# buwantaiji/DominantSparseEigenAD

Hardware: AMD Instinct MI355X
Metric: DominantSparseSymeig fwd+bwd ms & HBM GB/s (TFIM, fp64) (higher is better)
Workload: dtype f64

## Files before the change

dominantsparseeigenad_amd/csrc/dsea_capi.hip:

```cpp
#include <hip/hip_runtime.h>
#include <stdint.h>
#include <stdlib.h>
#include <string.h>

#include <new>

#include "dsea_internal.h"

using namespace dsea;

namespace {
thread_local int g_last_hip = 0;

inline int64_t round_up(int64_t v, int64_t m) { return (v + m - 1) / m * m; }

struct WsLayout {
  size_t partials_off, aux_off, coef_off, scal_off, vec_off, total;
  int64_t npad;
};
WsLayout ws_layout(int64_t n, int kmax) {
  WsLayout L;
  const int kk = kmax < 1 ? 1 : kmax;
  L.npad = round_up(n < 1 ? 1 : n, 256);
  size_t off = 0;
// ... 316 lines not shown
  REQUIRE(rows >= 1 && ld >= 8 && tau >= 0.0, DSEA_ERR_ARG);
  REQUIRE(aligned16(shadow_bf16) && (ld % 8) == 0, DSEA_ERR_ALIGN);
  drop_shadow8(ws->w);
  ws->w.shadow = static_cast<uint16_t*>(shadow_bf16);
  ws->w.shadow_ld = ld;
  ws->w.shadow_rows = rows;
  ws->w.lp_tau = tau;
  return DSEA_OK;
}

int dsea_ws_set_shadow8(dsea_ws_t ws, void* shadow_e5m2, int64_t ld, int rows, double tau) {
  REQUIRE(ws, DSEA_ERR_ARG);
  if (!shadow_e5m2) {
    drop_shadow8(ws->w);
    return DSEA_OK;
  }
  REQUIRE(rows >= 1 && ld >= 16 && tau >= 0.0, DSEA_ERR_ARG);
  REQUIRE(aligned16(shadow_e5m2) && (ld % 16) == 0, DSEA_ERR_ALIGN);
  drop_shadow(ws->w);
  ws->w.shadow8 = static_cast<uint8_t*>(shadow_e5m2);
  ws->w.shadow8_ld = ld;
  ws->w.shadow8_rows = rows;
  ws->w.lp8_tau = tau;
  return DSEA_OK;
}

ShadowRow Workspace::shadow_row(int row, int64_t n_rows) const {
  if (shadow && shadow_rows > row && shadow_ld >= n_rows) return ShadowRow(shadow + (int64_t)row * shadow_ld);
  if (shadow8 && shadow8_rows > row && shadow8_ld >= n_rows)
    return ShadowRow(shadow8 + (int64_t)row * shadow8_ld, shadow8_scale(n_rows));
  return ShadowRow();
}

int dsea_lanczos_lp_stats(dsea_ws_t ws, int64_t* lp_steps, int64_t* fp64_steps, void* stream) {
  REQUIRE(ws && lp_steps && fp64_steps, DSEA_ERR_ARG);
  double h[2] = {0.0, 0.0};
  DSEA_TRY(read_to_host(h, ws->w.scal + 16, sizeof(h), static_cast<hipStream_t>(stream)));
  *lp_steps = (int64_t)h[0];
  *fp64_steps = (int64_t)h[1];
  return DSEA_OK;
}

int dsea_lanczos_reorth_stats(dsea_ws_t ws, int64_t* reorth_steps, double* anorm, void* stream) {
  REQUIRE(ws && reorth_steps, DSEA_ERR_ARG);
  double h[2] = {0.0, 0.0};
  DSEA_TRY(read_to_host(h, ws->w.scal + DSEA_SCAL_PRO + 2, sizeof(h), static_cast<hipStream_t>(stream)));
  if (anorm) *anorm = h[0];
  *reorth_steps = (int64_t)h[1];
  return DSEA_OK;
}

int dsea_ws_set_rows_per_lane(dsea_ws_t ws, int rpl) {
  REQUIRE(ws && (rpl == 0 || rpl == 2 || rpl == 4 || rpl == 8 || rpl == 16), DSEA_ERR_ARG);
  ws->w.rpl_override = rpl;
  return DSEA_OK;
}

int dsea_ws_set_persist(dsea_ws_t ws, int mode) {
  REQUIRE(ws, DSEA_ERR_ARG);
  if (mode == 200) {
    ws->w.persist_override = mode;
    return DSEA_OK;
  }
  const int geo = mode >= 100 ? mode - 100 : mode;
  REQUIRE(geo == -1 || geo == 0 || geo == 1 || geo == 2 || geo == 11 || geo == 12 || geo == 21 || geo == 22, DSEA_ERR_ARG);
  REQUIRE(mode < 100 || geo != -1, DSEA_ERR_ARG);
// ... 399 lines not shown
                     int64_t n, void* stream) {
  (void)ws;
  REQUIRE(r && nrm2 && q_out && n >= 1, DSEA_ERR_ARG);
  REQUIRE(aligned16(r) && aligned16(q_out), DSEA_ERR_ALIGN);
  launch_scale_store(r, nrm2, q_out, beta_out, n, static_cast<hipStream_t>(stream));
  return check_launch();
}

int dsea_lanczos_rdots(dsea_ws_t ws, const double* Q, int64_t ldq, int64_t n, int i, const double* u,
                       const double* alpha, const double* beta, double* r, double* c_out, void* stream) {
  REQUIRE(ws && Q && u && alpha && r && c_out && n >= 1 && i >= 1 && ldq >= n, DSEA_ERR_ARG);
  REQUIRE(i <= ws->w.kmax, DSEA_ERR_WORKSPACE);
  REQUIRE(aligned16(Q) && aligned16(u) && aligned16(r) && (ldq % 2 == 0), DSEA_ERR_ALIGN);
  TileGeom g = ws->w.geom(n);
  Profiler* prof = ws->w.prof;
  launch_rdots(g, Q, ldq, n, i, u, alpha, beta, r, ws->w.partials, c_out, static_cast<hipStream_t>(stream),
               prof ? prof->next(PROF_RDOTS) : nullptr, nullptr, 0, nullptr, true);
  return check_launch();
}

int dsea_lanczos_axpy_norm(dsea_ws_t ws, const double* Q, int64_t ldq, int64_t n, int i, const double* c,
                           double* r, double* nrm2_out, void* stream) {
  REQUIRE(ws && Q && c && r && nrm2_out && n >= 1 && i >= 1 && ldq >= n, DSEA_ERR_ARG);
  REQUIRE(aligned16(Q) && aligned16(r) && (ldq % 2 == 0), DSEA_ERR_ALIGN);
  hipStream_t st = static_cast<hipStream_t>(stream);
  Workspace& w = ws->w;
  if (w.shadow && w.shadow_rows >= i && w.shadow_ld >= n && !w.geom(n).split_w) {
    double* nP = w.aux + DSEA_MAX_WAVE_TILES;
    const int rps = lp_rows_per_step(n, false);
    int nn = launch_axpy_norm_lp(n, rps, Q, ldq, w.shadow, w.shadow_ld, i, c, w.lp_tau, r, nP, w.scal + 16, st);
    launch_finalize1(nP, nn, nrm2_out, st);
  } else if (w.shadow8 && w.shadow8_rows >= i && w.shadow8_ld >= n && lp8_applies(n, w.geom(n).split_w != 0)) {
    double* nP = w.aux + DSEA_MAX_WAVE_TILES;
    int nn = launch_axpy_norm_lp8(n, Q, ldq, w.shadow8, w.shadow8_ld, shadow8_scale(n), i, c, w.lp8_tau, r, nP, w.scal + 16, st);
    launch_finalize1(nP, nn, nrm2_out, st);
  } else {
    TileGeom g = w.geom(n);
    launch_axpy_norm(g, Q, ldq, n, i, c, r, w.partials, nrm2_out, st);
  }
  return check_launch();
}

int dsea_lanczos_partial_step(dsea_ws_t ws, const double* Q, int64_t ldq, int64_t n, int i, const double* u,
                              const double* alphas, const double* betas, double* r, double* nrm2_out, void* stream) {
  REQUIRE(ws && Q && u && alphas && betas && r && nrm2_out && n >= 1 && i >= 1 && ldq >= n, DSEA_ERR_ARG);
  REQUIRE(i <= ws->w.kmax, DSEA_ERR_WORKSPACE);
  REQUIRE(aligned16(Q) && aligned16(u) && aligned16(r) && (ldq % 2 == 0), DSEA_ERR_ALIGN);
  hipStream_t st = static_cast<hipStream_t>(stream);
  Workspace& w = ws->w;
  REQUIRE(w.n >= n, DSEA_ERR_WORKSPACE);
  const TileGeom g = w.geom(n);
  double* flag = w.scal + DSEA_SCAL_PRO;
  double* om = w.aux + 4 * DSEA_MAX_WAVE_TILES;
  if (i == 1) HIP_TRY(hipMemsetAsync(flag, 0, 4 * sizeof(double), st));
  launch_rdots(g, Q, ldq, n, i, u, alphas + (i - 1), i >= 2 ? betas + (i - 2) : nullptr, r, w.partials, nullptr, st, nullptr,
               nullptr, 0, nullptr, true, nullptr, w.zero, false);
  launch_pro_update(alphas, betas, w.partials + (int64_t)i * g.pstride, rdots_partial_count(g, i), w.coef + i, om,
                    DSEA_MAX_WAVE_TILES, flag, flag + 1, i, 64.0 * 2.220446049250313e-16, w.pro_delta, nullptr, st);
  launch_rdots(g, Q, ldq, n, i, r, w.zero, nullptr, w.vec[2], w.partials, w.coef, st, nullptr, nullptr, 0, nullptr, false,
               nullptr, flag, true);
  launch_axpy_norm(g, Q, ldq, n, i, w.coef, r, w.partials, nrm2_out, st, nullptr, nullptr, flag);
  return check_launch();
}

int dsea_lanczos_store(dsea_ws_t ws, const double* r, const double* nrm2, double* Q, int64_t ldq, int row,
                       double* beta_out, int64_t n, void* stream) {
  REQUIRE(ws && r && nrm2 && Q && n >= 1 && row >= 0 && ldq >= n, DSEA_ERR_ARG);
// ... 219 lines not shown

int dsea_lanczos_run(dsea_op_t op, dsea_ws_t ws, int k, const double* q0, double* Q, int64_t ldq,
                     double* alphas, double* betas, void* stream) {
  REQUIRE(op && ws && q0 && Q && alphas && betas && k >= 1, DSEA_ERR_ARG);
  const int64_t n = op->d.n;
  REQUIRE(ldq >= n && ws->w.n >= n, DSEA_ERR_ARG);
  REQUIRE(k <= ws->w.kmax || k == 1, DSEA_ERR_WORKSPACE);
  REQUIRE(aligned16(q0) && aligned16(Q) && (ldq % 2 == 0), DSEA_ERR_ALIGN);
  hipStream_t st = static_cast<hipStream_t>(stream);
  Workspace& w = ws->w;
  double* P = w.partials;
  double* u = w.vec[0];
  double* r = w.vec[1];
  double* nrm2 = w.scal + 0;
  TileGeom g = w.geom(n);

  Profiler* prof = w.prof;
  uint16_t* Qs = nullptr;
  int64_t lds = 0;
  if (!w.partial_reorth && w.shadow && w.shadow_rows >= k && w.shadow_ld >= n && (!w.geom(n).split_w || n >= 32768)) {
    Qs = w.shadow;
    lds = w.shadow_ld;
  }
  uint8_t* Qs8 = nullptr;
  if (!w.partial_reorth && w.shadow8 && w.shadow8_rows >= k && w.shadow8_ld >= n && lp8_applies(n, g.split_w != 0))
    Qs8 = w.shadow8;
  const int64_t ld8 = w.shadow8_ld;
  const double scale8 = shadow8_scale(n);
  const bool lp = Qs || Qs8;
  auto shadow_row = [&](int i) -> ShadowRow {
    if (Qs8) return ShadowRow(Qs8 + (int64_t)i * ld8, scale8);
    return ShadowRow(Qs ? Qs + (int64_t)i * lds : nullptr);
  };
  double* lp_count = w.scal + 16;
  double* brk = w.scal + DSEA_SCAL_BREAK;
  HIP_TRY(hipMemsetAsync(lp_count, 0, (DSEA_SCAL_BREAK + 2 - 16) * sizeof(double), st));
  HIP_TRY(hipMemsetAsync(w.scal + DSEA_SCAL_LZ_FAIL, 0, (DSEA_SCAL_PRO + 4 - DSEA_SCAL_LZ_FAIL) * sizeof(double), st));
  if (w.lz_persist != 0 && w.reorth_passes == 1 && !w.partial_reorth && (w.lz_persist == 1 || n <= 4096) && !prof && lanczos_persist_applicable(op->d, n, k) &&
      lanczos_persist_comm_bytes(n, k) <= w.partials_bytes()) {
    const int rc = persist_status(launch_lanczos_persist(op->d, k, q0, Q, ldq, alphas, betas, brk, w.scal + DSEA_SCAL_LZ_FAIL, P,
                                                         st, w.lose_peer));
    if (rc != PERSIST_SKIPPED) return rc == DSEA_OK ? check_launch() : rc;
  }
  if (w.lz_persist != 0 && w.lz_persist != 2 && (w.lz_persist == 1 || (n >= 49152 && k <= 400)) && w.reorth_passes == 1 &&
      !w.partial_reorth && !prof && lanczos_persist_mid_applicable(op->d, n, k) &&
      lanczos_persist_mid_comm_bytes(n, k) <= w.partials_bytes()) {
    const int rc = persist_status(launch_lanczos_persist_mid(op->d, k, q0, Q, ldq, Qs, lds, w.lp_tau, alphas, betas, brk,
                                                             w.scal + DSEA_SCAL_LZ_FAIL, lp_count, P, st, w.lose_peer));
    if (rc != PERSIST_SKIPPED) return rc == DSEA_OK ? check_launch() : rc;
  }
  const int rps = lp_rows_per_step(n, g.split_w != 0);
  const bool fused_tail = has_fused_tail(op->d);
  if (w.partial_reorth && !fused_tail) return DSEA_ERR_UNSUPPORTED;
  double* aP = w.aux;
  double* nP = w.aux + DSEA_MAX_WAVE_TILES;
  auto correct = [&](int i, double* fp64P, EventPair* ev, bool close) -> int {
    int nn = g.nw;
    if (Qs8)
      nn = launch_axpy_norm_lp8(n, Q, ldq, Qs8, ld8, scale8, i, w.coef, w.lp8_tau, r, nP, lp_count, st, ev, brk);
    else if (Qs)
      nn = launch_axpy_norm_lp(n, rps, Q, ldq, Qs, lds, i, w.coef, w.lp_tau, r, nP, lp_count, st, ev, brk);
    else
      launch_axpy_norm(g, Q, ldq, n, i, w.coef, r, fp64P, nullptr, st, ev, brk);
    if (close) launch_finalize_slot(lp ? nP : fp64P, nn, nrm2, brk, st);
    return nn;
  };
  auto second_pass = [&](int i, double* fp64P, bool close, int& nn) -> int {
    HIP_TRY(hipMemcpyAsync(w.vec[2], r, (size_t)n * sizeof(double), hipMemcpyDeviceToDevice, st));
    launch_rdots(g, Q, ldq, n, i, w.vec[2], w.zero, nullptr, r, P, w.coef, st, nullptr, nullptr, 0, nullptr, lp, brk);
    nn = correct(i, fp64P, nullptr, close);
    return DSEA_OK;
  };
  launch_dot(q0, q0, n, P, nrm2, st);
  launch_scale_store(q0, nrm2, Q, nullptr, n, st, shadow_row(0));
  if (fused_tail) {
    int na = launch_spmv(op->d, Q, u, nullptr, nullptr, aP, st, prof ? prof->next(PROF_SPMV) : nullptr);
    if (na < 0) return DSEA_ERR_UNSUPPORTED;
    double* pro_flag = w.scal + DSEA_SCAL_PRO;
    double* pro_om = w.aux + 4 * DSEA_MAX_WAVE_TILES;
    const double pro_eps1 = 64.0 * 2.220446049250313e-16;
    for (int i = 1; i < k; ++i) {
      const double* beta_prev = (i >= 2) ? betas + (i - 2) : nullptr;
      if (w.partial_reorth) {
        launch_rdots(g, Q, ldq, n, i, u, nullptr, beta_prev, r, P, nullptr, st, nullptr, aP, na, alphas + (i - 1),
                     true, brk, w.zero, false);
        launch_pro_update(alphas, betas, P + (int64_t)i * g.pstride, rdots_partial_count(g, i), w.coef + i, pro_om,
                          DSEA_MAX_WAVE_TILES, pro_flag, pro_flag + 1, i, pro_eps1, w.pro_delta, brk, st);
        launch_rdots(g, Q, ldq, n, i, r, w.zero, nullptr, w.vec[2], P, w.coef, st,
                     prof ? prof->next(PROF_RDOTS) : nullptr, nullptr, 0, nullptr, false, brk, pro_flag, true);
        launch_axpy_norm(g, Q, ldq, n, i, w.coef, r, nP, nullptr, st, prof ? prof->next(PROF_AXPY) : nullptr, brk, pro_flag);
        na = launch_tfim_fused(op->d, r, nP, g.nw, Q + (int64_t)i * ldq, u, betas + (i - 1), aP, st,
                               prof ? prof->next(PROF_SPMV) : nullptr, nullptr, brk, i);
        continue;
      }
      launch_rdots(g, Q, ldq, n, i, u, nullptr, beta_prev, r, P, w.coef, st,
                   prof ? prof->next(PROF_RDOTS) : nullptr, aP, na, alphas + (i - 1), lp, brk);
      int nn = correct(i, nP, prof ? prof->next(PROF_AXPY) : nullptr, false);
      if (w.reorth_passes == 2) DSEA_TRY(second_pass(i, nP, false, nn));
      na = launch_tfim_fused(op->d, r, nP, nn, Q + (int64_t)i * ldq, u, betas + (i - 1), aP, st,
                             prof ? prof->next(PROF_SPMV) : nullptr, shadow_row(i), brk, i);
    }
    launch_finalize_slot(aP, na, alphas + (k - 1), brk, st);
    return check_launch();
  }
  int nb = launch_spmv(op->d, Q, u, nullptr, nullptr, P, st, prof ? prof->next(PROF_SPMV) : nullptr);
  if (nb < 0) return DSEA_ERR_UNSUPPORTED;
  launch_finalize1(P, nb, alphas, st);
  for (int i = 1; i < k; ++i) {
    const double* beta_prev = (i >= 2) ? betas + (i - 2) : nullptr;
    launch_rdots(g, Q, ldq, n, i, u, alphas + (i - 1), beta_prev, r, P, w.coef, st,
                 prof ? prof->next(PROF_RDOTS) : nullptr, nullptr, 0, nullptr, lp, brk);
    int nn = correct(i, P, prof ? prof->next(PROF_AXPY) : nullptr, true);
    if (w.reorth_passes == 2) DSEA_TRY(second_pass(i, P, true, nn));
    double* qi = Q + (int64_t)i * ldq;
    launch_scale_store(r, nrm2, qi, betas + (i - 1), n, st, shadow_row(i), brk, i);
    nb = launch_spmv(op->d, qi, u, nullptr, brk, P, st, prof ? prof->next(PROF_SPMV) : nullptr);
    launch_finalize_slot(P, nb, alphas + i, brk, st);
  }
  return check_launch();
}

int dsea_lanczos_run_basisfree(dsea_op_t op, dsea_ws_t ws, int k, const double* q0, double* Qrot, int64_t ldq,
                               double* alphas, double* betas, const double* s, double* psi, void* stream) {
  REQUIRE(op && ws && q0 && Qrot && alphas && betas && k >= 1 && ((s == nullptr) == (psi == nullptr)), DSEA_ERR_ARG);
  const int64_t n = op->d.n;
  REQUIRE(ldq >= n && ws->w.n >= n, DSEA_ERR_ARG);
  REQUIRE(aligned16(q0) && aligned16(Qrot) && (!psi || aligned16(psi)) && (ldq % 2 == 0), DSEA_ERR_ALIGN);
  REQUIRE(has_fused_tail(op->d), DSEA_ERR_UNSUPPORTED);
  hipStream_t st = static_cast<hipStream_t>(stream);
  Workspace& w = ws->w;
  double* u = w.vec[0];
  double* r = w.vec[1];
  double* nrm2 = w.scal + 0;
  double* aP = w.aux;
  double* nP = w.aux + DSEA_MAX_WAVE_TILES;
  double* brk = w.scal + DSEA_SCAL_BREAK;
  HIP_TRY(hipMemsetAsync(brk, 0, 2 * sizeof(double), st));
  HIP_TRY(hipMemsetAsync(w.scal + DSEA_SCAL_LZ_FAIL, 0, sizeof(double), st));
  if (psi) HIP_TRY(hipMemsetAsync(psi, 0, (size_t)n * sizeof(double), st));
  auto slot = [&](int i) { return Qrot + (int64_t)(i % 3) * ldq; };
  launch_dot(q0, q0, n, w.partials, nrm2, st);
  launch_scale_store(q0, nrm2, slot(0), nullptr, n, st, nullptr);
  int na = launch_spmv(op->d, slot(0), u, nullptr, nullptr, aP, st);
  if (na < 0) return DSEA_ERR_UNSUPPORTED;
// ... 364 lines not shown
```

dominantsparseeigenad_amd/csrc/dsea_internal.h:

```cpp
#ifndef DSEA_INTERNAL_H
#define DSEA_INTERNAL_H

#include <hip/hip_ext.h>
#include <hip/hip_runtime.h>
#include <stdint.h>

#include <functional>
#include <type_traits>

#include "../../include/dsea.h"

#define DSEA_MAX_EW_BLOCKS 2048
#define DSEA_MAX_WAVE_TILES 8192
#define DSEA_TFIM_TILE_LOG2 11
#define DSEA_MAX_TFIM_BLOCKS 4096
#define DSEA_PERSIST_MAX_TILES 4096
#define DSEA_MAX_KRYLOV 8000
#define DSEA_PERSIST_CG_MAX_TILES 1024
#define DSEA_SCALARS 64
#define DSEA_SCAL_BREAK 20
#define DSEA_SCAL_PRO 40
#define DSEA_PRO_DELTA_DEFAULT 1e-10
#define DSEA_SCAL_LZ_FAIL 38

// ... 75 lines not shown
  const double* c;
};
struct LatticeDesc {
  int L, nb;
  const double* c;
  uint8_t a[DSEA_LATTICE_MAX_BONDS], b[DSEA_LATTICE_MAX_BONDS];
};
enum OpKind { OP_TFIM = 1, OP_CSR = 2, OP_STENCIL3 = 3, OP_SELL = 4, OP_DENSE = 5, OP_TRANSFER = 6, OP_SYMDENSE = 7, OP_CHAIN = 8,
              OP_LATTICE = 9 };
struct OpDesc {
  OpKind kind;
  int64_t n;
  int tune_tile_log2;
  int tune_csr_group;
  int tune_sell_unroll;
  TfimParams tfim;
  CsrParams csr;
  Stencil3Params st3;
  SellParams sell;
  DenseParams dense;
  TransferParams transfer;
  SymDenseParams symdense;
  ChainParams chain;
  LatticeDesc lattice;
};

struct ShadowRow {
  uint16_t* h;
  uint8_t* b;
  double S;
  ShadowRow(uint16_t* bf16 = nullptr) : h(bf16), b(nullptr), S(0.0) {}
  ShadowRow(uint8_t* e5m2, double scale) : h(nullptr), b(e5m2), S(scale) {}
};

struct TileGeom {
  int rpl;
  int nw;
  int64_t ntiles;
  int pstride;
  int split_w;
  int dots_w;
  int dots_nt;
};

template <int V>
using int_c = std::integral_constant<int, V>;
template <int V, int... Rest, class F>
inline void dispatch_int(int v, F&& f) {
  if constexpr (sizeof...(Rest) == 0) {
    f(int_c<V>{});
  } else {
    if (v == V) f(int_c<V>{});
    else dispatch_int<Rest...>(v, f);
  }
}
template <class F>
inline void dispatch_bool(bool b, F&& f) {
  if (b) f(std::true_type{});
  else f(std::false_type{});
}
template <class F>
inline void dispatch_rpl(int rpl, F&& f) { dispatch_int<2, 4, 8, 16>(rpl, f); }
template <class F>
inline void dispatch_split_w(int w, F&& f) { dispatch_int<4, 8, 16>(w, f); }

enum ProfKind { PROF_RDOTS = 0, PROF_AXPY = 1, PROF_SPMV = 2, PROF_KINDS = 3 };
// ... 19 lines not shown
  }
};

struct Workspace {
  int64_t n, npad;
  int kmax;
  int rpl_override;
  int split_override;
  int persist_override;
  int lz_persist;
  int arnoldi_optimistic;
  int last_cg_form;
  int lose_peer;
  int reorth_passes;
  int partial_reorth;
  double pro_delta;
  double* partials;
  double* aux;
  double* coef;
  double* coef2;
  double* zero;
  double* scal;
  double* vec[4];
  Profiler* prof;
  uint16_t* shadow;
  int64_t shadow_ld;
  int shadow_rows;
  double lp_tau;
  uint8_t* shadow8;
  int64_t shadow8_ld;
  int shadow8_rows;
  double lp8_tau;
  ShadowRow shadow_row(int row, int64_t n) const;
  int callable_na;
  int defer_norm;
  const double* pend_P;
  int pend_count;
  double* pend_out;
  TileGeom geom(int64_t n_rows) const;
  size_t partials_bytes() const { return (size_t)DSEA_MAX_WAVE_TILES * (size_t)((kmax < 1 ? 1 : kmax) + 1) * sizeof(double); }
  size_t aux_bytes() const { return (size_t)4 * DSEA_MAX_WAVE_TILES * sizeof(double); }
};

inline int ew_blocks(int64_t n) {
  int64_t nb = (n + 2047) / 2048;
  if (nb < 1) nb = 1;
  if (nb > DSEA_MAX_EW_BLOCKS) nb = DSEA_MAX_EW_BLOCKS;
  return (int)nb;
}
inline int tile_blocks(int64_t n) {
  const int64_t nt = (n + 511) / 512;
  return nt <= DSEA_PERSIST_MAX_TILES ? (int)(nt < 1 ? 1 : nt) : ew_blocks(n);
}

void launch_finalize1(const double* P, int count, double* out, hipStream_t st);
int launch_three_term(const double* u, const double* q1, const double* q2, const double* aP, int aCount,
                      double* a_store, const double* beta, double* r, double* P, double* psi, const double* s1,
                      int64_t n, double* brk, hipStream_t st);
void launch_finalize_slot(const double* P, int count, double* out, const double* skip, hipStream_t st);
void launch_rdots(const TileGeom& g, const double* Q, int64_t ldq, int64_t n, int i, const double* u,
                  const double* alpha, const double* beta, double* r, double* P, double* c_out,
                  hipStream_t st, EventPair* ev = nullptr, const double* aP = nullptr, int aCount = 0,
                  double* a_store = nullptr, bool want_rr = false, double* brk = nullptr,
                  const double* sel = nullptr, bool sel_exit = false, const double* uscale = nullptr);
inline bool rdots_uscale_ok(const TileGeom& g) { return g.split_w == 0; }
int launch_axpy_norm_lp(int64_t n, int rps, const double* Q, int64_t ldq, const uint16_t* Qs, int64_t lds, int i,
                        const double* c, double tau, double* r, double* P, double* lp_count, hipStream_t st,
                        EventPair* ev = nullptr, const double* brk = nullptr);
int launch_axpy_norm_lp8(int64_t n, const double* Q, int64_t ldq, const uint8_t* Qs8, int64_t ld8, double scale, int i,
                         const double* c, double tau, double* r, double* P, double* lp_count, hipStream_t st,
                         EventPair* ev = nullptr, const double* brk = nullptr);
inline double shadow8_scale(int64_t n) {
  int e = 0;
  while (e < 15 && ((int64_t)1 << (2 * e)) < n) ++e;
  return (double)((int64_t)1 << e);
}
int launch_tfim_fused(const OpDesc& op, const double* r, const double* nP, int nCount, double* q_out, double* y,
                      double* beta_store, double* P, hipStream_t st, EventPair* ev = nullptr,
                      ShadowRow qs_out = ShadowRow(), double* brk = nullptr, int step = 0);
int launch_cg_update_fused(double* x, double* r, const double* d, const double* Ad, const double* state,
                           int parity, const double* dP, int dCount, int64_t n, double* P, hipStream_t st);
void launch_cg_direction_fused(const double* r, double* d, double* state, int parity, const double* rP,
                               int rCount, double eps, int64_t n, hipStream_t st);
void launch_axpy_norm(const TileGeom& g, const double* Q, int64_t ldq, int64_t n, int i, const double* c,
                      double* r, double* P, double* nrm2_out, hipStream_t st, EventPair* ev = nullptr,
                      const double* brk = nullptr, const double* sel = nullptr);
void launch_ritz(const TileGeom& g, const double* Q, int64_t ldq, int64_t n, int k, const double* s,
                 double* out, hipStream_t st);
void launch_dot(const double* x, const double* y, int64_t n, double* P, double* out, hipStream_t st);
void launch_pro_update(const double* alphas, const double* betas, const double* rrP, int rrCount, double* rr_store,
                       double* om, int ld, double* flag, double* state, int i, double eps1, double delta,
                       const double* brk, hipStream_t st);
int rdots_partial_count(const TileGeom& g, int i);
void launch_probe(const double* x, double* y, int64_t n, double* P, int nP, hipStream_t st);
void launch_shift_dot(const double* x, double* y, const double* shift, const double* skip, int64_t n,
                      double* P, double* out, hipStream_t st);
int launch_shift_dot_partials(const double* x, double* y, const double* shift, const double* skip, int64_t n, double* P,
                              hipStream_t st);
void launch_axpy(double a_host, const double* a_dev, const double* x, double* y, int64_t n, hipStream_t st);
void launch_scale_store(const double* r, const double* nrm2, double* q, double* beta_out, int64_t n,
                        hipStream_t st, ShadowRow qs = ShadowRow(), double* brk = nullptr, int step = 0);
void launch_scale_store_fused(const double* r, const double* nP, int nCount, double* q, ShadowRow qs, double* beta_store,
                              int64_t n, hipStream_t st);
int launch_dot_partials(const double* x, const double* y, int64_t n, double* P, hipStream_t st);
// ... 150 lines not shown
```

dominantsparseeigenad_amd/csrc/dsea_lanczos_kernels.hip:

```cpp

#include <hip/hip_runtime.h>
#include <stdint.h>

#include "dsea_internal.h"
#include "dsea_device.h"

namespace dsea {

__global__ __launch_bounds__(256) void k_finalize1(const double* __restrict__ partials, int count,
                                                   double* __restrict__ out) {
  __shared__ double sm4[4];
  double acc = 0.0;
  for (int b = threadIdx.x; b < count; b += 256) acc += partials[b];
  double t = block_sum(acc, sm4);
  if (threadIdx.x == 0) out[0] = t;
}

void launch_finalize1(const double* P, int count, double* out, hipStream_t st) {
  hipLaunchKernelGGL(k_finalize1, dim3(1), dim3(256), 0, st, P, count, out);
}

__global__ __launch_bounds__(256) void k_finalize_pair(const double* __restrict__ PA, int na, double* __restrict__ outA,
                                                       const double* __restrict__ PB, int nb, double* __restrict__ outB,
                                                       const double* __restrict__ skipB) {
  __shared__ double sm4[4];
  const bool second = blockIdx.x == 1;
  if (second && skipB && skipB[0] != 0.0) return;
  const double* __restrict__ P = second ? PB : PA;
  const int count = second ? nb : na;
  double acc = 0.0;
  for (int b = threadIdx.x; b < count; b += 256) acc += P[b];
  double t = block_sum(acc, sm4);
  if (threadIdx.x == 0) (second ? outB : outA)[0] = t;
}

void launch_finalize_pair(const double* PA, int na, double* outA, const double* PB, int nb, double* outB,
                          const double* skipB, hipStream_t st) {
  hipLaunchKernelGGL(k_finalize_pair, dim3(2), dim3(256), 0, st, PA, na, outA, PB, nb, outB, skipB);
}

template <bool GATE>
__global__ __launch_bounds__(256) void k_finalize_multi(const double* __restrict__ P, int64_t pstride,
                                                        int nw, double* __restrict__ c,
                                                        const double* __restrict__ brk,
                                                        const double* __restrict__ gate) {
  __shared__ double sm4[4];
  const double gate0 = GATE ? gate[0] : 1.0;
  if (broken(brk)) return;
  if (GATE && gate0 == 0.0) return;
  const int j = blockIdx.x;
  const double* __restrict__ row = P + (int64_t)j * pstride;
  double a0 = 0.0, a1 = 0.0, a2 = 0.0, a3 = 0.0;
  int w = threadIdx.x;
  for (; w + 768 < nw; w += 1024) {
    a0 += row[w];
    a1 += row[w + 256];
    a2 += row[w + 512];
    a3 += row[w + 768];
  }
  for (; w < nw; w += 256) a0 += row[w];
  double t = block_sum((a0 + a1) + (a2 + a3), sm4);
  if (threadIdx.x == 0) c[j] = t;
}

template <int NP>
struct RdotsPre {
  double2 uu[NP], qa[NP], qb[NP];
};

template <int RPL, bool GUARD, bool PRE, bool USCALE = false>
__device__ __forceinline__ void rdots_tile(const double* __restrict__ Q, int64_t ldq, int i, int ii, int64_t n,
                                           int64_t base, int lane, const double* __restrict__ u,
                                           double a, double b, double* __restrict__ r,
                                           double* __restrict__ sP, bool accumulate, bool want_rr,
                                           const RdotsPre<RPL / 2>& pre, double usc = 1.0) {
  constexpr int NP = RPL / 2;
  double2 rv[NP];
  const double* __restrict__ q1 = Q + (int64_t)(i - 1) * ldq;
  const double* __restrict__ q2 = (i >= 2) ? Q + (int64_t)(i - 2) * ldq : nullptr;
#pragma unroll
  for (int t = 0; t < NP; ++t) {
    const int64_t row = base + t * 128 + lane * 2;
    double2 uu, qa, qb;
    if (PRE) {
      uu = pre.uu[t];
      qa = pre.qa[t];
      qb = pre.qb[t];
    } else {
      uu = ld2<GUARD>(u, row, n);
      qa = ld2<GUARD>(q1, row, n);
      qb = make_double2(0.0, 0.0);
      if (q2) qb = ld2<GUARD>(q2, row, n);
    }
    if (USCALE) {
      uu.x = uu.x / usc;
// ... 314 lines not shown
  part[wv][lane] = w;
  __syncthreads();
  if (wv == 0) {
    double2 tot = part[0][lane];
#pragma unroll
    for (int k2 = 1; k2 < W; ++k2) {
      tot.x += part[k2][lane].x;
      tot.y += part[k2][lane].y;
    }
    if (MODE == 0) {
      double2 rv = ld2<true>(r, row, n);
      rv.x -= tot.x;
      rv.y -= tot.y;
      st2<true>(r, row, n, rv);
      double acc = wave_sum(fma(rv.x, rv.x, rv.y * rv.y));
      if (lane == 0) P[tile] = acc;
    } else {
      st2<true>(r, row, n, tot);
    }
  }
}

static inline int rdots_waves_per_block(int i) { return (i + 1) <= 2048 ? 4 : ((i + 1) <= 4096 ? 2 : 1); }

int rdots_partial_count(const TileGeom& g, int i) {
  if (g.split_w) return (int)((g.ntiles + g.dots_nt - 1) / g.dots_nt);
  const int wpb = rdots_waves_per_block(i);
  return (g.nw + wpb - 1) / wpb;
}

void launch_rdots(const TileGeom& g, const double* Q, int64_t ldq, int64_t n, int i, const double* u,
                  const double* alpha, const double* beta, double* r, double* P, double* c_out,
                  hipStream_t st, EventPair* ev, const double* aP, int aCount, double* a_store, bool want_rr,
                  double* brk, const double* sel, bool sel_exit, const double* uscale) {
  const int wr = want_rr ? 1 : 0;
  const int count = rdots_partial_count(g, i);
  if (g.split_w) {
    const size_t lds = (size_t)(i + 1) * sizeof(double);
    auto go = [&](auto w, auto nt) {
      dispatch_bool(sel != nullptr, [&](auto s) {
        constexpr int W = decltype(w)::value;
        constexpr bool SEL = decltype(s)::value;
        klaunch(ev, k_rdots_split<W, decltype(nt)::value, SEL>, count, W * 64, lds, st, Q, ldq, i, n, u, alpha, beta, r,
                P, g.pstride, aP, aCount, a_store, wr, brk, sel, SEL && sel_exit ? 1 : 0);
      });
    };
    if (g.dots_nt == 2) go(int_c<16>{}, int_c<2>{});
    else dispatch_split_w(g.dots_w, [&](auto w) { go(w, int_c<1>{}); });
  } else {
    const int wpb = rdots_waves_per_block(i);
    const size_t lds = (size_t)wpb * (i + 1) * sizeof(double);
    dispatch_int<1, 2, 0>(sel ? 1 : (uscale ? 2 : 0), [&](auto variant) {
      dispatch_rpl(g.rpl, [&](auto rpl) {
        constexpr bool SEL = decltype(variant)::value == 1, USCALE = decltype(variant)::value == 2;
        klaunch(ev, k_rdots<decltype(rpl)::value, SEL, USCALE>, count, 64 * wpb, lds, st, Q, ldq, i, n, u, alpha, beta, r,
                P, g.pstride, g.nw, g.ntiles, aP, aCount, a_store, wr, brk, sel, !USCALE && sel_exit ? 1 : 0,
                USCALE ? uscale : nullptr);
      });
    });
  }
  if (c_out)
    dispatch_bool(sel_exit, [&](auto gate) {
      constexpr bool GATE = decltype(gate)::value;
      klaunch(nullptr, k_finalize_multi<GATE>, want_rr ? i + 1 : i, 256, 0, st, P, g.pstride, count, c_out, brk,
              GATE ? sel : nullptr);
    });
}

template <int MODE>
static void launch_axpy_family(const TileGeom& g, const double* Q, int64_t ldq, int64_t n, int i, const double* c,
                               double* r, double* P, hipStream_t st, EventPair* ev, const double* brk,
                               const double* sel) {
  auto go = [&](auto s) {
    constexpr bool SEL = decltype(s)::value;
    if (g.split_w)
      dispatch_split_w(g.split_w, [&](auto w) {
        constexpr int W = decltype(w)::value;
        klaunch(ev, k_axpy_norm_split<W, MODE, SEL>, (unsigned)g.ntiles, W * 64, 0, st, Q, ldq, i, n, c, r, P, brk, sel);
      });
    else
      dispatch_rpl(g.rpl, [&](auto rpl) {
        klaunch(ev, k_axpy_norm<decltype(rpl)::value, MODE, SEL>, (g.nw + 3) / 4, 256, 0, st, Q, ldq, i, n, c, r, P, g.nw,
                g.ntiles, brk, sel);
      });
  };
  if constexpr (MODE == 0) dispatch_bool(sel != nullptr, go);
  else go(std::false_type{});
}

void launch_axpy_norm(const TileGeom& g, const double* Q, int64_t ldq, int64_t n, int i, const double* c,
                      double* r, double* P, double* nrm2_out, hipStream_t st, EventPair* ev, const double* brk,
                      const double* sel) {
  launch_axpy_family<0>(g, Q, ldq, n, i, c, r, P, st, ev, brk, sel);
  if (nrm2_out) launch_finalize1(P, g.nw, nrm2_out, st);
}

void launch_ritz(const TileGeom& g, const double* Q, int64_t ldq, int64_t n, int k, const double* s,
                 double* out, hipStream_t st) {
// ... 195 lines not shown
      st2<true>(r, row + 2 * t, n, rv);
      acc = fma(rv.x, rv.x, acc);
      acc = fma(rv.y, rv.y, acc);
    }
    acc = wave_sum(acc);
    if (lane == 0) P[tile] = acc;
  }
}

int launch_axpy_norm_lp(int64_t n, int rps, const double* Q, int64_t ldq, const uint16_t* Qs, int64_t lds, int i,
                        const double* c, double tau, double* r, double* P, double* lp_count, hipStream_t st,
                        EventPair* ev, const double* brk) {
  if (rps == 0) {
    const int64_t nt = (n + 511) / 512;
    klaunch(ev, k_axpy_norm_lp_split<16>, (unsigned)nt, 1024, 0, st, Q, ldq, Qs, lds, i, n, c, tau * tau, r, P, lp_count, brk);
    return (int)nt;
  }
  const int64_t tile = 512 * (int64_t)rps;
  int64_t ntiles = (n + tile - 1) / tile;
  if (ntiles < 1) ntiles = 1;
  const int nw = (int)(ntiles < DSEA_MAX_WAVE_TILES ? ntiles : DSEA_MAX_WAVE_TILES);
  dispatch_int<1, 2>(rps, [&](auto rows) {
    klaunch(ev, k_axpy_norm_lp<decltype(rows)::value>, (nw + 3) / 4, 256, 0, st, Q, ldq, Qs, lds, i, n, c, tau * tau, r, P,
            nw, ntiles, lp_count, brk);
  });
  return nw;
}

typedef float dsea_v2f __attribute__((ext_vector_type(2)));
__device__ __forceinline__ void fma_e5m2x4(dsea_v2f& w01, dsea_v2f& w23, dsea_v2f ch, uint32_t x) {
  w01 = __builtin_elementwise_fma(ch, __builtin_amdgcn_cvt_pk_f32_bf8((int)x, false), w01);
  w23 = __builtin_elementwise_fma(ch, __builtin_amdgcn_cvt_pk_f32_bf8((int)x, true), w23);
}
template <int RPS, bool GUARD>
__device__ __forceinline__ double axpy_lp8_tile(const uint8_t* __restrict__ Qs8, int64_t ld8, int i, int64_t n, int64_t base,
                                                int lane, const double* __restrict__ c, double cs, double rnorm,
                                                double* __restrict__ r) {
  dsea_v2f w[RPS][8];
#pragma unroll
  for (int s = 0; s < RPS; ++s)
#pragma unroll
    for (int e = 0; e < 8; ++e) w[s][e] = (dsea_v2f)(0.0f);
#ifndef DSEA_LP8_UNROLL
#define DSEA_LP8_UNROLL 8
#endif
#pragma unroll DSEA_LP8_UNROLL
  for (int jj = 0; jj < i; ++jj) {
    const int j = i - 1 - jj;
    const uint8_t* __restrict__ qj = Qs8 + (int64_t)j * ld8;
    const float chf = (float)(c[j] * cs);
    const dsea_v2f ch = (dsea_v2f)(chf);
#pragma unroll
    for (int s = 0; s < RPS; ++s) {
      const int64_t row = base + s * 1024 + lane * 16;
      uint4 h;
      if (!GUARD || row + 16 <= n) {
        h = ld_u4_stream(qj + row);
      } else {
        uint32_t t[4] = {0u, 0u, 0u, 0u};
        for (int e = 0; e < 16; ++e)
          if (row + e < n) t[e >> 2] |= (uint32_t)qj[row + e] << ((e & 3) * 8);
        h = make_uint4(t[0], t[1], t[2], t[3]);
      }
      fma_e5m2x4(w[s][0], w[s][1], ch, h.x);
      fma_e5m2x4(w[s][2], w[s][3], ch, h.y);
      fma_e5m2x4(w[s][4], w[s][5], ch, h.z);
      fma_e5m2x4(w[s][6], w[s][7], ch, h.w);
    }
  }
  double acc = 0.0;
#pragma unroll
  for (int s = 0; s < RPS; ++s) {
    const int64_t row = base + s * 1024 + lane * 16;
#pragma unroll
    for (int t = 0; t < 8; ++t) {
      double2 rv = ld2<GUARD>(r, row + 2 * t, n);
      rv.x = fma(-(double)w[s][t].x, rnorm, rv.x);
      rv.y = fma(-(double)w[s][t].y, rnorm, rv.y);
      st2<GUARD>(r, row + 2 * t, n, rv);
      acc = fma(rv.x, rv.x, acc);
      acc = fma(rv.y, rv.y, acc);
    }
  }
  return acc;
}
template <int RPS, bool GUARD>
__device__ __forceinline__ double axpy_lp8_tile_fp64(const double* __restrict__ Q, int64_t ldq, int i, int64_t n, int64_t base,
                                                     int lane, const double* __restrict__ c, double* __restrict__ r) {
  double2 w[RPS * 8];
#pragma unroll
  for (int t = 0; t < RPS * 8; ++t) w[t] = make_double2(0.0, 0.0);
  for (int jj = 0; jj < i; ++jj) {
    const int j = i - 1 - jj;
    const double* __restrict__ qj = Q + (int64_t)j * ldq;
    const double cj = c[j];
#pragma unroll
    for (int t = 0; t < RPS * 8; ++t) {
      const double2 q = ld2_stream<GUARD>(qj, base + t * 128 + lane * 2, n);
      w[t].x = fma(cj, q.x, w[t].x);
      w[t].y = fma(cj, q.y, w[t].y);
    }
  }
  double acc = 0.0;
#pragma unroll
  for (int t = 0; t < RPS * 8; ++t) {
    const int64_t row = base + t * 128 + lane * 2;
    double2 rv = ld2<GUARD>(r, row, n);
    rv.x -= w[t].x;
    rv.y -= w[t].y;
    st2<GUARD>(r, row, n, rv);
    acc = fma(rv.x, rv.x, acc);
    acc = fma(rv.y, rv.y, acc);
  }
  return acc;
}

template <int RPS>
__global__ __launch_bounds__(256) void k_axpy_norm_lp8(const double* __restrict__ Q, int64_t ldq,
                                                       const uint8_t* __restrict__ Qs8, int64_t ld8, double scale, int i,
                                                       int64_t n, const double* __restrict__ c, double tau2,
                                                       double* __restrict__ r, double* __restrict__ P, int nw,
                                                       int64_t ntiles, double* __restrict__ lp_count,
                                                       const double* __restrict__ brk) {
  const int lane = threadIdx.x & 63;
  const int64_t widx = (int64_t)blockIdx.x * 4 + (threadIdx.x >> 6);
  if (widx >= nw) return;
  if (broken(brk)) return;
  double m = 0.0;
  for (int b = lane; b < i; b += 64) {
    const double v = c[b];
    m = fmax(m, v * v);
  }
  m = wave_max(m);
  const double rr = c[i];
  const bool use_lp = m <= tau2 * rr;
  if (widx == 0 && lane == 0 && lp_count) lp_count[use_lp ? 0 : 1] += 1.0;
  const double rnorm = sqrt(rr);
  const double cs = rnorm > 0.0 ? 1.0 / (scale * rnorm) : 0.0;
  constexpr int64_t TILE = 1024 * RPS;
  double acc = 0.0;
  for (int64_t tile = widx; tile < ntiles; tile += nw) {
    const int64_t base = tile * TILE;
    const bool whole = base + TILE <= n;
    if (use_lp)
      acc += whole ? axpy_lp8_tile<RPS, false>(Qs8, ld8, i, n, base, lane, c, cs, rnorm, r)
                   : axpy_lp8_tile<RPS, true>(Qs8, ld8, i, n, base, lane, c, cs, rnorm, r);
    else
      acc += whole ? axpy_lp8_tile_fp64<RPS, false>(Q, ldq, i, n, base, lane, c, r)
                   : axpy_lp8_tile_fp64<RPS, true>(Q, ldq, i, n, base, lane, c, r);
  }
  acc = wave_sum(acc);
  if (lane == 0) P[widx] = acc;
}

int launch_axpy_norm_lp8(int64_t n, const double* Q, int64_t ldq, const uint8_t* Qs8, int64_t ld8, double scale, int i,
                         const double* c, double tau, double* r, double* P, double* lp_count, hipStream_t st,
                         EventPair* ev, const double* brk) {
#ifndef DSEA_LP8_RPS
#define DSEA_LP8_RPS 1
#endif
  constexpr int RPS = DSEA_LP8_RPS;
  const int64_t tile = 1024 * (int64_t)RPS;
  int64_t ntiles = (n + tile - 1) / tile;
  if (ntiles < 1) ntiles = 1;
  const int nw = (int)(ntiles < DSEA_MAX_WAVE_TILES ? ntiles : DSEA_MAX_WAVE_TILES);
  klaunch(ev, k_axpy_norm_lp8<RPS>, (nw + 3) / 4, 256, 0, st, Q, ldq, Qs8, ld8, scale, i, n, c, tau * tau, r, P, nw, ntiles,
          lp_count, brk);
  return nw;
}

__global__ __launch_bounds__(256) void k_pro_update(const double* __restrict__ alphas, const double* __restrict__ betas,
                                                    const double* __restrict__ rrP, int rrCount,
                                                    double* __restrict__ rr_store, double* __restrict__ om, int ld,
                                                    double* __restrict__ flag, double* __restrict__ state, int i,
                                                    double eps1, double delta, const double* __restrict__ brk) {
  __shared__ double smax[256];
  __shared__ double sm5[5];
  const double a = alphas[i - 1];
  const double bprev = (i >= 2) ? betas[i - 2] : 0.0;
  const double anorm_prev = state[1];
  const double rr = sum_partials_block(rrP, rrCount, sm5);
  if (broken(brk)) return;
  if (threadIdx.x == 0) rr_store[0] = rr;
  const double bcur = sqrt(rr);
  const double anorm = fmax(anorm_prev, fabs(a) + bcur + bprev);
  double* __restrict__ o1 = om + (size_t)((i - 1) & 1) * ld;
  double* __restrict__ o2 = om + (size_t)(i & 1) * ld;
  double mx = 0.0;
  for (int k = threadIdx.x; k <= i - 1; k += 256) {
    double v;
    if (k == i - 1) {
      v = eps1 * anorm / bcur;
    } else {
      const double w1k = o1[k];
      const double w1p = (k + 1 == i - 1) ? 1.0 : o1[k + 1];
      const double w1m = (k > 0) ? o1[k - 1] : 0.0;
      const double w2k = (k == i - 2) ? 1.0 : o2[k];
      double t = betas[k] * w1p + (alphas[k] - a) * w1k - bprev * w2k;
      if (k > 0) t += betas[k - 1] * w1m;
      const double d = eps1 * ((betas[k] + bcur) + anorm);
// ... 68 lines not shown
```

Measured before the change: 6502.

## Precompute lp8 gate and scaled fp32 coefficients once in finalize last-block

Moves the per-wave computation of the low-precision gate (max coefficient vs residual norm), rnorm and the scaled float coefficients out of the e5m2 axpy-norm kernel. The last block to finish the rdots finalize, found through an atomic ticket, now writes a flag and a float coefficient array that every wave reads. Without that fused path, a separate one-block prepare kernel is launched. This removes redundant per-wave reductions and per-row double-to-float conversions, at the cost of an atomic ticket, a grid-wide fence and an extra launch on the unfused path.

```diff
diff --git a/dominantsparseeigenad_amd/csrc/dsea_capi.hip b/dominantsparseeigenad_amd/csrc/dsea_capi.hip
--- a/dominantsparseeigenad_amd/csrc/dsea_capi.hip
+++ b/dominantsparseeigenad_amd/csrc/dsea_capi.hip
@@ -372,6 +372,16 @@
   return ShadowRow();
 }
 
+Lp8Prep Workspace::lp8_prep(int64_t n_rows) const {
+  Lp8Prep p;
+  p.scale = shadow8_scale(n_rows);
+  p.tau2 = lp8_tau * lp8_tau;
+  p.flag = coef2;
+  p.chat = reinterpret_cast<float*>(coef2 + 2);
+  p.ticket = reinterpret_cast<unsigned*>(scal + DSEA_SCAL_LP8_TICKET);
+  return p;
+}
+
 int dsea_lanczos_lp_stats(dsea_ws_t ws, int64_t* lp_steps, int64_t* fp64_steps, void* stream) {
   REQUIRE(ws && lp_steps && fp64_steps, DSEA_ERR_ARG);
   double h[2] = {0.0, 0.0};
@@ -837,7 +847,9 @@
     launch_finalize1(nP, nn, nrm2_out, st);
   } else if (w.shadow8 && w.shadow8_rows >= i && w.shadow8_ld >= n && lp8_applies(n, w.geom(n).split_w != 0)) {
     double* nP = w.aux + DSEA_MAX_WAVE_TILES;
-    int nn = launch_axpy_norm_lp8(n, Q, ldq, w.shadow8, w.shadow8_ld, shadow8_scale(n), i, c, w.lp8_tau, r, nP, w.scal + 16, st);
+    REQUIRE(i <= w.kmax, DSEA_ERR_WORKSPACE);
+    int nn = launch_axpy_norm_lp8(n, Q, ldq, w.shadow8, w.shadow8_ld, shadow8_scale(n), i, c, w.lp8_tau, r, nP, w.scal + 16,
+                                  w.lp8_prep(n), false, st);
     launch_finalize1(nP, nn, nrm2_out, st);
   } else {
     TileGeom g = w.geom(n);
@@ -1123,9 +1135,12 @@
     if (Qs8) return ShadowRow(Qs8 + (int64_t)i * ld8, scale8);
     return ShadowRow(Qs ? Qs + (int64_t)i * lds : nullptr);
   };
+  const Lp8Prep prep8 = w.lp8_prep(n);
+  const Lp8Prep* prep = Qs8 && lp8_prepared() ? &prep8 : nullptr;
   double* lp_count = w.scal + 16;
   double* brk = w.scal + DSEA_SCAL_BREAK;
   HIP_TRY(hipMemsetAsync(lp_count, 0, (DSEA_SCAL_BREAK + 2 - 16) * sizeof(double), st));
+  if (prep) HIP_TRY(hipMemsetAsync(prep8.ticket, 0, sizeof(double), st));
   HIP_TRY(hipMemsetAsync(w.scal + DSEA_SCAL_LZ_FAIL, 0, (DSEA_SCAL_PRO + 4 - DSEA_SCAL_LZ_FAIL) * sizeof(double), st));
   if (w.lz_persist != 0 && w.reorth_passes == 1 && !w.partial_reorth && (w.lz_persist == 1 || n <= 4096) && !prof && lanczos_persist_applicable(op->d, n, k) &&
       lanczos_persist_comm_bytes(n, k) <= w.partials_bytes()) {
@@ -1148,7 +1163,8 @@
   auto correct = [&](int i, double* fp64P, EventPair* ev, bool close) -> int {
     int nn = g.nw;
     if (Qs8)
-      nn = launch_axpy_norm_lp8(n, Q, ldq, Qs8, ld8, scale8, i, w.coef, w.lp8_tau, r, nP, lp_count, st, ev, brk);
+      nn = launch_axpy_norm_lp8(n, Q, ldq, Qs8, ld8, scale8, i, w.coef, w.lp8_tau, r, nP, lp_count, prep8, prep != nullptr, st, ev,
+                                brk);
     else if (Qs)
       nn = launch_axpy_norm_lp(n, rps, Q, ldq, Qs, lds, i, w.coef, w.lp_tau, r, nP, lp_count, st, ev, brk);
     else
@@ -1158,7 +1174,8 @@
   };
   auto second_pass = [&](int i, double* fp64P, bool close, int& nn) -> int {
     HIP_TRY(hipMemcpyAsync(w.vec[2], r, (size_t)n * sizeof(double), hipMemcpyDeviceToDevice, st));
-    launch_rdots(g, Q, ldq, n, i, w.vec[2], w.zero, nullptr, r, P, w.coef, st, nullptr, nullptr, 0, nullptr, lp, brk);
+    launch_rdots(g, Q, ldq, n, i, w.vec[2], w.zero, nullptr, r, P, w.coef, st, nullptr, nullptr, 0, nullptr, lp, brk, nullptr,
+                 false, nullptr, prep);
     nn = correct(i, fp64P, nullptr, close);
     return DSEA_OK;
   };
@@ -1185,7 +1202,7 @@
         continue;
       }
       launch_rdots(g, Q, ldq, n, i, u, nullptr, beta_prev, r, P, w.coef, st,
-                   prof ? prof->next(PROF_RDOTS) : nullptr, aP, na, alphas + (i - 1), lp, brk);
+                   prof ? prof->next(PROF_RDOTS) : nullptr, aP, na, alphas + (i - 1), lp, brk, nullptr, false, nullptr, prep);
       int nn = correct(i, nP, prof ? prof->next(PROF_AXPY) : nullptr, false);
       if (w.reorth_passes == 2) DSEA_TRY(second_pass(i, nP, false, nn));
       na = launch_tfim_fused(op->d, r, nP, nn, Q + (int64_t)i * ldq, u, betas + (i - 1), aP, st,
@@ -1200,7 +1217,7 @@
   for (int i = 1; i < k; ++i) {
     const double* beta_prev = (i >= 2) ? betas + (i - 2) : nullptr;
     launch_rdots(g, Q, ldq, n, i, u, alphas + (i - 1), beta_prev, r, P, w.coef, st,
-                 prof ? prof->next(PROF_RDOTS) : nullptr, nullptr, 0, nullptr, lp, brk);
+                 prof ? prof->next(PROF_RDOTS) : nullptr, nullptr, 0, nullptr, lp, brk, nullptr, false, nullptr, prep);
     int nn = correct(i, P, prof ? prof->next(PROF_AXPY) : nullptr, true);
     if (w.reorth_passes == 2) DSEA_TRY(second_pass(i, P, true, nn));
     double* qi = Q + (int64_t)i * ldq;
diff --git a/dominantsparseeigenad_amd/csrc/dsea_internal.h b/dominantsparseeigenad_amd/csrc/dsea_internal.h
--- a/dominantsparseeigenad_amd/csrc/dsea_internal.h
+++ b/dominantsparseeigenad_amd/csrc/dsea_internal.h
@@ -131,6 +131,14 @@
   ShadowRow(uint16_t* bf16 = nullptr) : h(bf16), b(nullptr), S(0.0) {}
   ShadowRow(uint8_t* e5m2, double scale) : h(nullptr), b(e5m2), S(scale) {}
 };
+
+struct Lp8Prep {
+  double scale, tau2;
+  double* flag;
+  float* chat;
+  unsigned* ticket;
+};
+#define DSEA_SCAL_LP8_TICKET 48
 
 struct TileGeom {
   int rpl;
@@ -216,6 +224,7 @@
   int shadow8_rows;
   double lp8_tau;
   ShadowRow shadow_row(int row, int64_t n) const;
+  Lp8Prep lp8_prep(int64_t n) const;
   int callable_na;
   int defer_norm;
   const double* pend_P;
@@ -236,6 +245,8 @@
   const int64_t nt = (n + 511) / 512;
   return nt <= DSEA_PERSIST_MAX_TILES ? (int)(nt < 1 ? 1 : nt) : ew_blocks(n);
 }
+
+bool lp8_prepared();
 
 void launch_finalize1(const double* P, int count, double* out, hipStream_t st);
 int launch_three_term(const double* u, const double* q1, const double* q2, const double* aP, int aCount,
@@ -246,14 +257,15 @@
                   const double* alpha, const double* beta, double* r, double* P, double* c_out,
                   hipStream_t st, EventPair* ev = nullptr, const double* aP = nullptr, int aCount = 0,
                   double* a_store = nullptr, bool want_rr = false, double* brk = nullptr,
-                  const double* sel = nullptr, bool sel_exit = false, const double* uscale = nullptr);
+                  const double* sel = nullptr, bool sel_exit = false, const double* uscale = nullptr,
+                  const Lp8Prep* prep = nullptr);
 inline bool rdots_uscale_ok(const TileGeom& g) { return g.split_w == 0; }
 int launch_axpy_norm_lp(int64_t n, int rps, const double* Q, int64_t ldq, const uint16_t* Qs, int64_t lds, int i,
                         const double* c, double tau, double* r, double* P, double* lp_count, hipStream_t st,
                         EventPair* ev = nullptr, const double* brk = nullptr);
 int launch_axpy_norm_lp8(int64_t n, const double* Q, int64_t ldq, const uint8_t* Qs8, int64_t ld8, double scale, int i,
-                         const double* c, double tau, double* r, double* P, double* lp_count, hipStream_t st,
-                         EventPair* ev = nullptr, const double* brk = nullptr);
+                         const double* c, double tau, double* r, double* P, double* lp_count, const Lp8Prep& prep, bool prepared,
+                         hipStream_t st, EventPair* ev = nullptr, const double* brk = nullptr);
 inline double shadow8_scale(int64_t n) {
   int e = 0;
   while (e < 15 && ((int64_t)1 << (2 * e)) < n) ++e;
diff --git a/dominantsparseeigenad_amd/csrc/dsea_lanczos_kernels.hip b/dominantsparseeigenad_amd/csrc/dsea_lanczos_kernels.hip
--- a/dominantsparseeigenad_amd/csrc/dsea_lanczos_kernels.hip
+++ b/dominantsparseeigenad_amd/csrc/dsea_lanczos_kernels.hip
@@ -39,12 +39,42 @@
   hipLaunchKernelGGL(k_finalize_pair, dim3(2), dim3(256), 0, st, PA, na, outA, PB, nb, outB, skipB);
 }
 
+template <bool COHERENT>
+__device__ __forceinline__ double lp8_ldc(const double* p) {
+  return COHERENT ? __hip_atomic_load(p, __ATOMIC_RELAXED, __HIP_MEMORY_SCOPE_AGENT) : *p;
+}
+template <bool COHERENT>
+__device__ __forceinline__ void lp8_prepare(const double* c, int i, const Lp8Prep& prep) {
+  const int lane = threadIdx.x & 63;
+  double m = 0.0;
+  for (int b = lane; b < i; b += 64) {
+    const double v = lp8_ldc<COHERENT>(c + b);
+    m = fmax(m, v * v);
+  }
+  m = wave_max(m);
+  const double rr = lp8_ldc<COHERENT>(c + i);
+  const bool use_lp = m <= prep.tau2 * rr;
+  const double rnorm = sqrt(rr);
+  const double cs = rnorm > 0.0 ? 1.0 / (prep.scale * rnorm) : 0.0;
+  for (int j = threadIdx.x; j < i; j += 256) prep.chat[j] = (float)(lp8_ldc<COHERENT>(c + j) * cs);
+  if (threadIdx.x == 0) {
+    prep.flag[0] = use_lp ? 1.0 : 0.0;
+    prep.flag[1] = rnorm;
+  }
+}
+__global__ __launch_bounds__(256) void k_lp8_prepare(const double* __restrict__ c, int i, Lp8Prep prep,
+                                                     const double* __restrict__ brk) {
+  if (broken(brk)) return;
+  lp8_prepare<false>(c, i, prep);
+}
+
 template <bool GATE>
 __global__ __launch_bounds__(256) void k_finalize_multi(const double* __restrict__ P, int64_t pstride,
                                                         int nw, double* __restrict__ c,
                                                         const double* __restrict__ brk,
-                                                        const double* __restrict__ gate) {
+                                                        const double* __restrict__ gate, Lp8Prep prep) {
   __shared__ double sm4[4];
+  __shared__ int last;
   const double gate0 = GATE ? gate[0] : 1.0;
   if (broken(brk)) return;
   if (GATE && gate0 == 0.0) return;
@@ -61,6 +91,18 @@
   for (; w < nw; w += 256) a0 += row[w];
   double t = block_sum((a0 + a1) + (a2 + a3), sm4);
   if (threadIdx.x == 0) c[j] = t;
+  if (prep.ticket) {
+    if (threadIdx.x == 0) {
+      __threadfence();
+      last = atomicAdd(prep.ticket, 1u) == gridDim.x - 1;
+    }
+    __syncthreads();
+    if (last) {
+      __threadfence();
+      lp8_prepare<true>(c, (int)gridDim.x - 1, prep);
+      if (threadIdx.x == 0) *prep.ticket = 0u;
+    }
+  }
 }
 
 template <int NP>
@@ -441,7 +483,7 @@
 void launch_rdots(const TileGeom& g, const double* Q, int64_t ldq, int64_t n, int i, const double* u,
                   const double* alpha, const double* beta, double* r, double* P, double* c_out,
                   hipStream_t st, EventPair* ev, const double* aP, int aCount, double* a_store, bool want_rr,
-                  double* brk, const double* sel, bool sel_exit, const double* uscale) {
+                  double* brk, const double* sel, bool sel_exit, const double* uscale, const Lp8Prep* prep) {
   const int wr = want_rr ? 1 : 0;
   const int count = rdots_partial_count(g, i);
   if (g.split_w) {
@@ -472,7 +514,7 @@
     dispatch_bool(sel_exit, [&](auto gate) {
       constexpr bool GATE = decltype(gate)::value;
       klaunch(nullptr, k_finalize_multi<GATE>, want_rr ? i + 1 : i, 256, 0, st, P, g.pstride, count, c_out, brk,
-              GATE ? sel : nullptr);
+              GATE ? sel : nullptr, prep && want_rr ? *prep : Lp8Prep{});
     });
 }
 
@@ -734,42 +776,45 @@
   w01 = __builtin_elementwise_fma(ch, __builtin_amdgcn_cvt_pk_f32_bf8((int)x, false), w01);
   w23 = __builtin_elementwise_fma(ch, __builtin_amdgcn_cvt_pk_f32_bf8((int)x, true), w23);
 }
-template <int RPS, bool GUARD>
-__device__ __forceinline__ double axpy_lp8_tile(const uint8_t* __restrict__ Qs8, int64_t ld8, int i, int64_t n, int64_t base,
-                                                int lane, const double* __restrict__ c, double cs, double rnorm,
-                                                double* __restrict__ r) {
-  dsea_v2f w[RPS][8];
-#pragma unroll
-  for (int s = 0; s < RPS; ++s)
-#pragma unroll
-    for (int e = 0; e < 8; ++e) w[s][e] = (dsea_v2f)(0.0f);
+template <int RPS, bool GUARD, bool PREP>
+__device__ __forceinline__ void lp8_vector(dsea_v2f (&w)[RPS][8], const uint8_t* __restrict__ Qs8, int64_t ld8, int j, int64_t n,
+                                           int64_t base, int lane, const double* __restrict__ c, double cs,
+                                           const float* __restrict__ chat) {
+  const uint8_t* __restrict__ qj = Qs8 + (int64_t)j * ld8;
+  const float chf = PREP ? chat[j] : (float)(c[j] * cs);
+  const dsea_v2f ch = (dsea_v2f)(chf);
+#pragma unroll
+  for (int s = 0; s < RPS; ++s) {
+    const int64_t row = base + s * 1024 + lane * 16;
+    uint4 h;
+    if (!GUARD || row + 16 <= n) {
+      h = ld_u4_stream(qj + row);
+    } else {
+      uint32_t t[4] = {0u, 0u, 0u, 0u};
+      for (int e = 0; e < 16; ++e)
+        if (row + e < n) t[e >> 2] |= (uint32_t)qj[row + e] << ((e & 3) * 8);
+      h = make_uint4(t[0], t[1], t[2], t[3]);
+    }
+    fma_e5m2x4(w[s][0], w[s][1], ch, h.x);
+    fma_e5m2x4(w[s][2], w[s][3], ch, h.y);
+    fma_e5m2x4(w[s][4], w[s][5], ch, h.z);
+    fma_e5m2x4(w[s][6], w[s][7], ch, h.w);
+  }
+}
 #ifndef DSEA_LP8_UNROLL
 #define DSEA_LP8_UNROLL 8
 #endif
+template <int RPS, bool GUARD, bool PREP>
+__device__ __forceinline__ double axpy_lp8_tile(const uint8_t* __restrict__ Qs8, int64_t ld8, int i, int64_t n, int64_t base,
+                                                int lane, const double* __restrict__ c, double cs, double rnorm,
+                                                const float* __restrict__ chat, double* __restrict__ r) {
+  dsea_v2f w[RPS][8];
+#pragma unroll
+  for (int s = 0; s < RPS; ++s)
+#pragma unroll
+    for (int e = 0; e < 8; ++e) w[s][e] = (dsea_v2f)(0.0f);
 #pragma unroll DSEA_LP8_UNROLL
-  for (int jj = 0; jj < i; ++jj) {
-    const int j = i - 1 - jj;
-    const uint8_t* __restrict__ qj = Qs8 + (int64_t)j * ld8;
-    const float chf = (float)(c[j] * cs);
-    const dsea_v2f ch = (dsea_v2f)(chf);
-#pragma unroll
-    for (int s = 0; s < RPS; ++s) {
-      const int64_t row = base + s * 1024 + lane * 16;
-      uint4 h;
-      if (!GUARD || row + 16 <= n) {
-        h = ld_u4_stream(qj + row);
-      } else {
-        uint32_t t[4] = {0u, 0u, 0u, 0u};
-        for (int e = 0; e < 16; ++e)
-          if (row + e < n) t[e >> 2] |= (uint32_t)qj[row + e] << ((e & 3) * 8);
-        h = make_uint4(t[0], t[1], t[2], t[3]);
-      }
-      fma_e5m2x4(w[s][0], w[s][1], ch, h.x);
-      fma_e5m2x4(w[s][2], w[s][3], ch, h.y);
-      fma_e5m2x4(w[s][4], w[s][5], ch, h.z);
-      fma_e5m2x4(w[s][6], w[s][7], ch, h.w);
-    }
-  }
+  for (int jj = 0; jj < i; ++jj) lp8_vector<RPS, GUARD, PREP>(w, Qs8, ld8, i - 1 - jj, n, base, lane, c, cs, chat);
   double acc = 0.0;
 #pragma unroll
   for (int s = 0; s < RPS; ++s) {
@@ -817,36 +862,56 @@
   return acc;
 }
 
-template <int RPS>
+struct Lp8Head {
+  bool use_lp;
+  double rnorm, cs;
+};
+template <bool PREP>
+__device__ __forceinline__ Lp8Head lp8_head(const double* __restrict__ c, int i, double scale, double tau2, double2 rec, int lane) {
+  Lp8Head h;
+  if (PREP) {
+    h.use_lp = rec.x != 0.0;
+    h.rnorm = rec.y;
+    h.cs = 0.0;
+    return h;
+  }
+  double m = 0.0;
+  for (int b = lane; b < i; b += 64) {
+    const double v = c[b];
+    m = fmax(m, v * v);
+  }
+  m = wave_max(m);
+  const double rr = c[i];
+  h.use_lp = m <= tau2 * rr;
+  h.rnorm = sqrt(rr);
+  h.cs = h.rnorm > 0.0 ? 1.0 / (scale * h.rnorm) : 0.0;
+  return h;
+}
+
+template <int RPS, bool PREP>
 __global__ __launch_bounds__(256) void k_axpy_norm_lp8(const double* __restrict__ Q, int64_t ldq,
                                                        const uint8_t* __restrict__ Qs8, int64_t ld8, double scale, int i,
                                                        int64_t n, const double* __restrict__ c, double tau2,
+                                                       const double* __restrict__ rec, const float* __restrict__ chat,
                                                        double* __restrict__ r, double* __restrict__ P, int nw,
                                                        int64_t ntiles, double* __restrict__ lp_count,
                                                        const double* __restrict__ brk) {
   const int lane = threadIdx.x & 63;
   const int64_t widx = (int64_t)blockIdx.x * 4 + (threadIdx.x >> 6);
   if (widx >= nw) return;
+  const double2 rec2 = PREP ? *reinterpret_cast<const double2*>(rec) : make_double2(0.0, 0.0);
   if (broken(brk)) return;
-  double m = 0.0;
-  for (int b = lane; b < i; b += 64) {
-    const double v = c[b];
-    m = fmax(m, v * v);
-  }
-  m = wave_max(m);
-  const double rr = c[i];
-  const bool use_lp = m <= tau2 * rr;
+  const Lp8Head hd = lp8_head<PREP>(c, i, scale, tau2, rec2, lane);
+  const bool use_lp = hd.use_lp;
   if (widx == 0 && lane == 0 && lp_count) lp_count[use_lp ? 0 : 1] += 1.0;
-  const double rnorm = sqrt(rr);
-  const double cs = rnorm > 0.0 ? 1.0 / (scale * rnorm) : 0.0;
   constexpr int64_t TILE = 1024 * RPS;
   double acc = 0.0;
   for (int64_t tile = widx; tile < ntiles; tile += nw) {
     const int64_t base = tile * TILE;
     const bool whole = base + TILE <= n;
     if (use_lp)
-      acc += whole ? axpy_lp8_tile<RPS, false>(Qs8, ld8, i, n, base, lane, c, cs, rnorm, r)
-                   : axpy_lp8_tile<RPS, true>(Qs8, ld8, i, n, base, lane, c, cs, rnorm, r);
+      acc += whole ? axpy_lp8_tile<RPS, false, PREP>(Qs8, ld8, i, n, base, lane, c, hd.cs, hd.rnorm, chat, r)
+                   : axpy_lp8_tile<RPS, true, PREP>(Qs8, ld8, i, n, base, lane, c, hd.cs, hd.rnorm, chat, r);
     else
       acc += whole ? axpy_lp8_tile_fp64<RPS, false>(Q, ldq, i, n, base, lane, c, r)
                    : axpy_lp8_tile_fp64<RPS, true>(Q, ldq, i, n, base, lane, c, r);
@@ -855,9 +920,14 @@
   if (lane == 0) P[widx] = acc;
 }
 
+bool lp8_prepared() {
+  const char* env = getenv("DSEA_LP8_PREPARED");
+  return !(env && env[0] == '0' && env[1] == 0);
+}
+
 int launch_axpy_norm_lp8(int64_t n, const double* Q, int64_t ldq, const uint8_t* Qs8, int64_t ld8, double scale, int i,
-                         const double* c, double tau, double* r, double* P, double* lp_count, hipStream_t st,
-                         EventPair* ev, const double* brk) {
+                         const double* c, double tau, double* r, double* P, double* lp_count, const Lp8Prep& prep, bool prepared,
+                         hipStream_t st, EventPair* ev, const double* brk) {
 #ifndef DSEA_LP8_RPS
 #define DSEA_LP8_RPS 1
 #endif
@@ -866,8 +936,14 @@
   int64_t ntiles = (n + tile - 1) / tile;
   if (ntiles < 1) ntiles = 1;
   const int nw = (int)(ntiles < DSEA_MAX_WAVE_TILES ? ntiles : DSEA_MAX_WAVE_TILES);
-  klaunch(ev, k_axpy_norm_lp8<RPS>, (nw + 3) / 4, 256, 0, st, Q, ldq, Qs8, ld8, scale, i, n, c, tau * tau, r, P, nw, ntiles,
-          lp_count, brk);
+  if (!lp8_prepared()) {
+    klaunch(ev, k_axpy_norm_lp8<RPS, false>, (nw + 3) / 4, 256, 0, st, Q, ldq, Qs8, ld8, scale, i, n, c, tau * tau, nullptr,
+            nullptr, r, P, nw, ntiles, lp_count, brk);
+    return nw;
+  }
+  if (!prepared) klaunch(nullptr, k_lp8_prepare, 1, 256, 0, st, c, i, prep, brk);
+  klaunch(ev, k_axpy_norm_lp8<RPS, true>, (nw + 3) / 4, 256, 0, st, Q, ldq, Qs8, ld8, scale, i, n, c, tau * tau, prep.flag,
+          prep.chat, r, P, nw, ntiles, lp_count, brk);
   return nw;
 }
 
```

Measured after the change: 6327. 0.973x the previous value.
